# dashpay/agora-blsful

Measured on NVIDIA B200. Metric: verified sigs/sec, 1M-batch G2Impl, higher is better.
Workload: dtype u32 limbs (381-bit modular integers)

## Files before the change

### agora-blsful_b200/csrc/blsgpu.cu

```cuda
#include <cuda_runtime.h>
#include <nvtx3/nvToolsExt.h>
#include <sys/random.h>

#include <algorithm>
#include <atomic>
#include <functional>
#include <cstdio>
#include <cstdlib>
#include <cstring>
#include <memory>
#include <mutex>
#include <string>
#include <unordered_map>
#include <thread>
#include <vector>

#include "../../include/blsgpu.h"
#include "kernels.cuh"

using namespace bls;

namespace {

thread_local std::string g_create_error;
// ... 770 lines not shown
  return BLSGPU_OK;
}

template <class PkA, class SigA>
size_t pipeline_other_bytes(size_t n) {
  typedef typename PtInfo<SigA>::Jac SigJ;
  size_t total = levels_total(make_levels(std::max<size_t>(n, 1)));
  size_t gtotal = levels_total(make_levels((std::max<size_t>(n, 1) + M6_GROUP - 1) / M6_GROUP));
  return gtotal * (sizeof(Fp12) + sizeof(SigJ)) + n * (sizeof(SigJ) + sizeof(Fp12) + sizeof(SigJ)) + total * sizeof(Digest) +
         n * (16 + 4 * 32) + ((size_t)32 << 16) * (12 + 2 * sizeof(SigJ)) + (1 << 20) + (n + 64) * 8 + 16 * 256 + 4096 +
         probe_scratch_bytes<PkA, SigA>(probe_cap((n + M6_GROUP - 1) / M6_GROUP)) +
         (n >= MSM_MIN_ITEMS ? (n / 96 + 2) * 32 * sizeof(SigJ) + std::min<size_t>(n / 384 + 1, 592) * 128 * NODE_BUCKETS * sizeof(SigJ) + n * 5 + 8 * 256 : 0);
}
size_t m6_line_bytes(size_t n, size_t chunk) {
  return (n > chunk ? 2 : 1) * std::max<size_t>(std::min(std::max<size_t>(n, 1), chunk), 6 * PROBE_SMALL) * M6_ITEM_BYTES;
}
int ensure_miller_arena(blsgpu_ctx* ctx, size_t n, size_t other) {
  plan_m6_chunk(ctx, n, other);
  for (;;) {
    const int r = ensure_arena(ctx, other + m6_line_bytes(n, ctx->m6_chunk));
    if (r != BLSGPU_E_ALLOC || ctx->m6_chunk <= M6_CHUNK_MIN || n <= M6_CHUNK_MIN) return r;
    (void)cudaGetLastError();
    ctx->m6_chunk = std::max(M6_CHUNK_MIN, std::min(ctx->m6_chunk, n) / 2 / 120 * 120);
  }
}
template <class PkA, class SigA>
int ensure_pipeline_arena(blsgpu_ctx* ctx, size_t n, size_t head_bytes) {
  return ensure_miller_arena(ctx, n, head_bytes + pipeline_other_bytes<PkA, SigA>(n));
}

template <class A>
int decode_points(blsgpu_ctx* ctx, size_t n, const uint8_t* d_in, int format, A* d_out, uint8_t* d_st, int kid = -1) {
  LAUNCH_TIMED(kid, (k_decode<A>), blocks_for(n), TPB, n, d_in, format, d_out, d_st);
  LAUNCH_TIMED(kid < 0 ? -1 : kid + 1, (k_subgroup_check<A>), blocks_for(n), TPB, n, d_out, d_st);
  return BLSGPU_OK;
}

struct Keys {
  const uint8_t* bytes = nullptr;
  KeySet* set = nullptr;
  const uint32_t* idx = nullptr;
  Keys(const uint8_t* b = nullptr) : bytes(b) {}
  Keys(KeySet* s, const uint32_t* i) : set(s), idx(i) {}
};
template <class PkA>
int load_keys(blsgpu_ctx* ctx, size_t n, const Keys& d_keys, int format, PkA* d_pk, uint8_t* d_st) {
  if (!d_keys.set) return decode_points<PkA>(ctx, n, d_keys.bytes, format, d_pk, d_st, BLSGPU_KERNEL_DECODE_PK);
  LAUNCH((k_gather_keys<PkA>), blocks_for(n), TPB, n, d_keys.idx, (const PkA*)d_keys.set->pts, (const uint8_t*)d_keys.set->st, d_pk, d_st);
  return BLSGPU_OK;
}

template <class HA, class PkA>
int hash_points(blsgpu_ctx* ctx, size_t n, const uint8_t* d_msgs, const uint64_t* d_moff, int msg_mode, const PkA* d_pk,
                const uint8_t* d_pre, const DstParam& dst, HA* d_h) {
  typedef typename PtInfo<HA>::Jac HJ;
  size_t mark = ctx->arena.off;
  HJ* d_hj = ctx->arena.take<HJ>(n);
  if (ctx->arena.off > ctx->arena.cap) {
    ctx->err = "hash_points: arena too small";
    return BLSGPU_E_ALLOC;
  }
  LAUNCH_TIMED(BLSGPU_KERNEL_HASH_MAP, (k_hash<HA, PkA>), blocks_for(n), TPB, n, d_msgs, d_moff, msg_mode, d_pk, d_pre, dst, d_hj);
  LAUNCH_TIMED(BLSGPU_KERNEL_CLEAR_COFACTOR, (k_clear_cofactor<HA>), blocks_for(n), TPB, n, d_hj);
  LAUNCH_TIMED(BLSGPU_KERNEL_TO_AFFINE, (k_to_affine_batch<HA>), blocks_for((n + TO_AFFINE_BATCH - 1) / TO_AFFINE_BATCH), TPB, n,
               (const HJ*)d_hj, d_h);
  ctx->arena.off = mark;
  return BLSGPU_OK;
}

template <int IMPL>
int verify_points_partials(blsgpu_ctx* ctx, Pipe<typename ImplT<IMPL>::PkAff, typename ImplT<IMPL>::SigAff>& P, int msg_mode, const DstParam& dst,
                           size_t n, const typename ImplT<IMPL>::PkAff* d_pk, const typename ImplT<IMPL>::SigAff* d_sig, const uint8_t* d_stpk,
                           const uint8_t* d_stsig, const uint8_t* d_msgs, const uint64_t* d_moff, uint8_t* d_status_out) {
  typedef typename ImplT<IMPL>::PkAff PkA;
  typedef typename ImplT<IMPL>::SigAff SigA;
  SigA* d_h = ctx->arena.take<SigA>(n);
  LAUNCH((k_prestatus<PkA, SigA>), blocks_for(n), TPB, n, d_stpk, d_stsig, d_pk, d_sig, d_status_out);
  stage_mark(ctx, BLSGPU_STAGE_HASH);
  CKR((hash_points<SigA, PkA>(ctx, n, d_msgs, d_moff, msg_mode, d_pk, (const uint8_t*)d_status_out, dst, d_h)));
  return pipeline_partials<PkA, SigA>(ctx, P, n, d_pk, d_sig, d_h, d_status_out, true);
}
template <int IMPL>
int verify_points(blsgpu_ctx* ctx, int msg_mode, const DstParam& dst, size_t n, const typename ImplT<IMPL>::PkAff* d_pk,
                  const typename ImplT<IMPL>::SigAff* d_sig, const uint8_t* d_stpk, const uint8_t* d_stsig, const uint8_t* d_msgs,
                  const uint64_t* d_moff, uint8_t* d_status_out) {
  typedef typename ImplT<IMPL>::PkAff PkA;
  typedef typename ImplT<IMPL>::SigAff SigA;
  Pipe<PkA, SigA> P;
  CKR((verify_points_partials<IMPL>(ctx, P, msg_mode, dst, n, d_pk, d_sig, d_stpk, d_stsig, d_msgs, d_moff, d_status_out)));
  return check_and_bisect(ctx, P);
}

template <int IMPL>
int verify_dev_partials(blsgpu_ctx* ctx, Pipe<typename ImplT<IMPL>::PkAff, typename ImplT<IMPL>::SigAff>& P, int msg_mode, const DstParam& dst,
                        int format, size_t n, const Keys& d_keys, const uint8_t* d_sigs, const uint8_t* d_msgs, const uint64_t* d_moff,
                        uint8_t* d_status_out) {
// ... 2612 lines not shown
```

### agora-blsful_b200/csrc/kernels.cuh

```cuda
#pragma once
#include <cuda_runtime.h>

#include "h2c.cuh"
#include "pairing.cuh"
#include "miller6.cuh"
#include "finalexp6.cuh"
#include "fr.cuh"

namespace bls {

template <class A>
struct PtInfo;
template <>
struct PtInfo<G1Aff> {
  static const int LEN = 48;
  typedef G1Jac Jac;
  typedef Fp F;
};
template <>
struct PtInfo<G2Aff> {
  static const int LEN = 96;
  typedef G2Jac Jac;
  typedef Fp2 F;
};
__device__ __forceinline__ uint8_t pt_decompress(G1Aff& r, const uint8_t* b, bool chk) { return g1_decompress(r, b, chk); }
__device__ __forceinline__ uint8_t pt_decompress(G2Aff& r, const uint8_t* b, bool chk) { return g2_decompress(r, b, chk); }
__device__ __forceinline__ void pt_compress(uint8_t* o, const G1Aff& p) { g1_compress(o, p); }
__device__ __forceinline__ void pt_compress(uint8_t* o, const G2Aff& p) { g2_compress(o, p); }
__device__ __forceinline__ void pt_generator(G1Aff& g) {
  fp_set(g.x, K_G1X);
  fp_set(g.y, K_G1Y);
  g.inf = 0;
}
__device__ __forceinline__ void pt_generator(G2Aff& g) {
  fp2_set(g.x, K_G2X);
  fp2_set(g.y, K_G2Y);
  g.inf = 0;
}
template <class A>
__device__ __forceinline__ void pt_set_inf(A& p) {
  fzero(p.x);
  fzero(p.y);
  p.inf = 1;
}

template <int IMPL>
struct ImplT;
template <>
struct ImplT<2> {
  typedef G1Aff PkAff;
  typedef G2Aff SigAff;
  typedef G1Jac PkJac;
  typedef G2Jac SigJac;
};
template <>
struct ImplT<1> {
  typedef G2Aff PkAff;
  typedef G1Aff SigAff;
  typedef G2Jac PkJac;
  typedef G1Jac SigJac;
};
__device__ __forceinline__ void hash_to_group(G2Jac& r, const uint8_t* pre, uint32_t pl, const uint8_t* m, uint32_t ml,
                                              const uint8_t* dst, uint32_t dl) {
  hash_to_g2(r, pre, pl, m, ml, dst, dl);
}
__device__ __forceinline__ void hash_to_group(G1Jac& r, const uint8_t* pre, uint32_t pl, const uint8_t* m, uint32_t ml,
                                              const uint8_t* dst, uint32_t dl) {
  hash_to_g1(r, pre, pl, m, ml, dst, dl);
}

__device__ __forceinline__ void hash_map_to_curve(G2Jac& r, const uint8_t* pre, uint32_t pl, const uint8_t* m, uint32_t ml,
                                                  const uint8_t* dst, uint32_t dl) {
  hash_map_g2(r, pre, pl, m, ml, dst, dl);
}
__device__ __forceinline__ void hash_map_to_curve(G1Jac& r, const uint8_t* pre, uint32_t pl, const uint8_t* m, uint32_t ml,
                                                  const uint8_t* dst, uint32_t dl) {
  hash_map_g1(r, pre, pl, m, ml, dst, dl);
}
__device__ __forceinline__ void clear_cofactor(G2Jac& r, const G2Jac& q) { g2_clear_cofactor(r, q); }
__device__ __forceinline__ void clear_cofactor(G1Jac& r, const G1Jac& q) { g1_clear_cofactor(r, q); }

struct DstParam {
  uint8_t b[64];
  uint32_t len;
};
struct Digest {
  uint8_t b[32];
};

#define BLS_TID() ((size_t)blockIdx.x * blockDim.x + threadIdx.x)
#ifndef BLS_MIN_BLOCKS
#define BLS_MIN_BLOCKS 1
#endif

#if !defined(BLS_SPLIT_MIN_BLOCKS)
#define BLS_SPLIT_MIN_BLOCKS 4
#endif
#if !defined(BLS_HASH_MIN_BLOCKS)
#define BLS_HASH_MIN_BLOCKS 3
#endif
#if !defined(BLS_SPLIT2_MIN_BLOCKS)
#define BLS_SPLIT2_MIN_BLOCKS 4
#endif
template <class A>
struct SplitBlocks {
  static constexpr int value = sizeof(A) > 2 * sizeof(Fp) + 16 ? BLS_SPLIT2_MIN_BLOCKS : BLS_SPLIT_MIN_BLOCKS;
};
#if !defined(BLS_MSM_MIN_BLOCKS)
#define BLS_MSM_MIN_BLOCKS 4
#endif
template <class A>
__global__ void __launch_bounds__(128, BLS_MIN_BLOCKS) k_decode(size_t n, const uint8_t* __restrict__ in, int format, A* __restrict__ out,
                                                uint8_t* __restrict__ st) {
  constexpr int L = PtInfo<A>::LEN;
  __shared__ __align__(16) uint8_t stage[128 * L];
  const size_t first = (size_t)blockIdx.x * blockDim.x;
  const size_t cnt = first < n ? (n - first < blockDim.x ? n - first : blockDim.x) : 0;
  const uint8_t* src = in + first * L;
  if ((reinterpret_cast<uintptr_t>(src) & 15u) == 0) {
    const uint4* v = reinterpret_cast<const uint4*>(src);
    uint4* d = reinterpret_cast<uint4*>(stage);
    const size_t quads = cnt * L / 16, tail = cnt * L - quads * 16;
    for (size_t q = threadIdx.x; q < quads; q += blockDim.x) d[q] = v[q];
    if (threadIdx.x < tail) stage[quads * 16 + threadIdx.x] = src[quads * 16 + threadIdx.x];
  } else {
    for (size_t b = threadIdx.x; b < cnt * L; b += blockDim.x) stage[b] = src[b];
  }
  __syncthreads();
  size_t i = BLS_TID();
  if (i >= n) return;
  uint8_t b[L];
  const uint32_t* rec = reinterpret_cast<const uint32_t*>(stage + threadIdx.x * L);
#pragma unroll
  for (int k = 0; k < L / 4; k++) {
    uint32_t w = rec[k];
    b[4 * k] = (uint8_t)w;
    b[4 * k + 1] = (uint8_t)(w >> 8);
    b[4 * k + 2] = (uint8_t)(w >> 16);
    b[4 * k + 3] = (uint8_t)(w >> 24);
  }
  uint8_t s = header_to_modern(b[0], format);
  A p;
  if (s == ST_OK) s = pt_decompress(p, b, false);
  if (s != ST_OK) pt_set_inf(p);
  out[i] = p;
  st[i] = s;
}

__device__ __forceinline__ bool pt_in_subgroup(const G1Aff& p) { return g1_in_subgroup(p); }
__device__ __forceinline__ bool pt_in_subgroup(const G2Aff& p) { return g2_in_subgroup(p); }
template <class A>
__global__ void __launch_bounds__(128, SplitBlocks<A>::value) k_subgroup_check(size_t n, A* __restrict__ pts, uint8_t* __restrict__ st) {
  size_t i = BLS_TID();
  if (i >= n || st[i] != ST_OK) return;
  A p = pts[i];
  if (p.inf || pt_in_subgroup(p)) return;
  pt_set_inf(p);
  pts[i] = p;
  st[i] = ST_DESERIALIZE;
}

template <class A>
__global__ void __launch_bounds__(128, BLS_MIN_BLOCKS) k_gather_keys(size_t n, const uint32_t* __restrict__ key_idx, const A* __restrict__ set_pts,
                                                     const uint8_t* __restrict__ set_st, A* __restrict__ out, uint8_t* __restrict__ st) {
  size_t i = BLS_TID();
  if (i >= n) return;
  const uint32_t k = key_idx[i];
  out[i] = set_pts[k];
  st[i] = set_st[k];
}

template <class A>
__global__ void __launch_bounds__(128, BLS_MIN_BLOCKS) k_encode(size_t n, const A* __restrict__ in, int format, uint8_t* __restrict__ out) {
  size_t i = BLS_TID();
  if (i >= n) return;
  constexpr int L = PtInfo<A>::LEN;
  uint8_t b[L];
  A p = in[i];
  pt_compress(b, p);
  header_from_modern(b[0], format);
  for (int k = 0; k < L; k++) out[i * L + k] = b[k];
}

template <class A>
__global__ void __launch_bounds__(128, BLS_MIN_BLOCKS) k_to_affine(size_t n, const typename PtInfo<A>::Jac* __restrict__ in, A* __restrict__ out) {
  size_t i = BLS_TID();
  if (i >= n) return;
  typename PtInfo<A>::Jac p = in[i];
  A a;
  jac_to_aff(a, p);
  out[i] = a;
}

#define TO_AFFINE_BATCH 16
template <class A>
__global__ void __launch_bounds__(128) k_to_affine_batch(size_t n, const typename PtInfo<A>::Jac* __restrict__ in, A* __restrict__ out) {
  size_t base = BLS_TID() * TO_AFFINE_BATCH;
  if (base >= n) return;
  size_t left = n - base;
  jac_to_aff_batch<typename PtInfo<A>::F, TO_AFFINE_BATCH>(out + base, in + base, left < TO_AFFINE_BATCH ? (int)left : TO_AFFINE_BATCH);
}

template <class PkA, class SigA>
__global__ void k_prestatus(size_t n, const uint8_t* st_pk, const uint8_t* st_sig, const PkA* pk, const SigA* sig,
                            uint8_t* out) {
  size_t i = BLS_TID();
  if (i >= n) return;
  uint8_t s = st_pk[i];
  if (s == ST_OK) s = st_sig[i];
  if (s == ST_OK && sig[i].inf) s = ST_SIG_IDENTITY;
  if (s == ST_OK && pk[i].inf) s = ST_PK_IDENTITY;
  out[i] = s;
}

template <class HA, class PkA>
__global__ void __launch_bounds__(128, BLS_HASH_MIN_BLOCKS) k_hash(size_t n, const uint8_t* __restrict__ msgs, const uint64_t* __restrict__ msg_off,
                                              int msg_mode, const PkA* __restrict__ pk, const uint8_t* __restrict__ pre,
                                              DstParam dst, typename PtInfo<HA>::Jac* __restrict__ out) {
  size_t i = BLS_TID();
  if (i >= n) return;
  typename PtInfo<HA>::Jac hj;
  if (pre != nullptr && pre[i] != ST_OK) {
    jac_set_inf(hj);
    out[i] = hj;
    return;
  }
  uint8_t prefix[PtInfo<PkA>::LEN];
  uint32_t plen = 0;
  if (msg_mode != 0) {
    PkA p = pk[i];
    pt_compress(prefix, p);
    plen = PtInfo<PkA>::LEN;
  }
  const uint8_t* m = msgs;
  uint32_t mlen = 0;
  if (msg_mode != 2) {
    uint64_t o0 = msg_off[i], o1 = msg_off[i + 1];
    m = msgs + o0;
    mlen = (uint32_t)(o1 - o0);
  }
  hash_map_to_curve(hj, prefix, plen, m, mlen, dst.b, dst.len);
  out[i] = hj;
}

template <class HA>
__global__ void __launch_bounds__(128, SplitBlocks<HA>::value) k_clear_cofactor(size_t n, typename PtInfo<HA>::Jac* __restrict__ pts) {
  size_t i = BLS_TID();
  if (i >= n) return;
  typename PtInfo<HA>::Jac q = pts[i], r;
  if (jac_is_inf(q)) return;
  clear_cofactor(r, q);
  pts[i] = r;
}

template <class P>
__device__ __forceinline__ void digest_point(Sha256& s, const P& p) {
  sha256_update(s, reinterpret_cast<const uint8_t*>(&p.x), sizeof(p.x));
  sha256_update(s, reinterpret_cast<const uint8_t*>(&p.y), sizeof(p.y));
  const uint8_t f = p.inf ? 1 : 0;
  sha256_update(s, &f, 1);
}
template <class PkA, class SigA>
__global__ void __launch_bounds__(128, BLS_MIN_BLOCKS) k_leaf_digest(size_t n, const PkA* pk, const SigA* sig, const SigA* h, Digest* out) {
  size_t i = BLS_TID();
  if (i >= n) return;
  Sha256 s;
  sha256_init(s);
  digest_point(s, pk[i]);
  digest_point(s, sig[i]);
  digest_point(s, h[i]);
  Digest d;
  sha256_final(s, d.b);
  out[i] = d;
}
__global__ void __launch_bounds__(128, BLS_MIN_BLOCKS) k_digest_reduce(size_t n_in, const Digest* in, size_t n_out, Digest* out) {
  size_t j = BLS_TID();
  if (j >= n_out) return;
  Sha256 s;
  sha256_init(s);
  for (int m = 0; m < 16; m++) {
    size_t idx = j + (size_t)m * n_out;
    if (idx < n_in) sha256_update(s, in[idx].b, 32);
  }
  Digest d;
  sha256_final(s, d.b);
// ... 460 lines not shown
__global__ void __launch_bounds__(128, BLS_MIN_BLOCKS) k_reduce_jac_w(size_t n_in, const J* __restrict__ in, size_t n_out, J* __restrict__ out) {
  const size_t t = BLS_TID(), j = t >> 4;
  const int m = (int)(t & 15);
  const size_t idx = j + (size_t)m * n_out;
  J acc;
  if (j < n_out && idx < n_in) acc = in[idx]; else jac_set_inf(acc);
#pragma unroll 1
  for (int s = 1; s < 16; s <<= 1) {
    J other;
    words_shfl_xor(other, acc, s);
    if ((m & (2 * s - 1)) == 0) jac_add(acc, acc, other);
  }
  if (j < n_out && m == 0) out[j] = acc;
}
template <class A>
__global__ void __launch_bounds__(128, BLS_MIN_BLOCKS) k_reduce_aff(size_t n_in, const A* __restrict__ in, size_t n_out,
                                                    typename PtInfo<A>::Jac* __restrict__ out) {
  size_t j = BLS_TID();
  if (j >= n_out) return;
  typename PtInfo<A>::Jac acc;
  jac_set_inf(acc);
  for (int m = 0; m < 16; m++) {
    size_t idx = j + (size_t)m * n_out;
    if (idx < n_in) {
      A t = in[idx];
      jac_add_mixed(acc, acc, t);
    }
  }
  out[j] = acc;
}

constexpr uint8_t PROBE_SKIP = 0xfe;
template <class PkA, class SigA>
__global__ void __launch_bounds__(128, BLS_MIN_BLOCKS) k_probe_fill_nodes(size_t cnt, const uint32_t* __restrict__ idx,
                                                          const typename PtInfo<SigA>::Jac* __restrict__ S, PkA* __restrict__ xpk,
                                                          SigA* __restrict__ xh, uint8_t* __restrict__ xpre) {
  size_t c = BLS_TID();
  if (c >= cnt) return;
  const size_t j = idx ? idx[c] : c;
  typename PtInfo<SigA>::Jac s = S[j];
  SigA sa;
  jac_to_aff(sa, s);
  PkA ng;
  pt_generator(ng);
  aff_neg(ng, ng);
  xpk[6 * c] = ng;
  xh[6 * c] = sa;
  xpre[6 * c] = sa.inf ? PROBE_SKIP : ST_OK;
  for (int m = 1; m < 6; m++) xpre[6 * c + m] = PROBE_SKIP;
}
template <class PkA, class SigA>
__global__ void __launch_bounds__(128, BLS_MIN_BLOCKS) k_probe_fill_leaves(size_t cnt, const uint32_t* __restrict__ idx, const PkA* __restrict__ pk,
                                                           const SigA* __restrict__ h, const SigA* __restrict__ sig,
                                                           const uint8_t* __restrict__ status, PkA* __restrict__ xpk,
                                                           SigA* __restrict__ xh, uint8_t* __restrict__ xpre) {
  size_t c = BLS_TID();
  if (c >= cnt) return;
  const size_t i = idx[c];
  const bool on = status[i] == ST_OK;
  if (on) {
    PkA ng;
    pt_generator(ng);
    aff_neg(ng, ng);
    xpk[6 * c] = pk[i];
    xh[6 * c] = h[i];
    xpk[6 * c + 1] = ng;
    xh[6 * c + 1] = sig[i];
// ... 798 lines not shown
```

### agora-blsful_b200/csrc/fp.cuh

```cuda
#pragma once
#include <stdint.h>

#if defined(__CUDACC__)
#define BLS_HD __device__ __forceinline__
#define BLS_FN __device__ __noinline__
#define BLS_CONST __device__ __constant__ const
#else
#define BLS_HD static inline
#define BLS_FN static
#define BLS_CONST static const
#endif

#include "consts_gen.h"

#if defined(BLS_TRACK)
#include <cstdio>
#include <cstdlib>
#include <execinfo.h>
#define BLS_REQ(cond, what)                                                                  \
  do {                                                                                       \
    if (!(cond)) {                                                                           \
      fprintf(stderr, "BLS_TRACK bound violation: %s (%s:%d)\n", what, __FILE__, __LINE__);  \
      void* bt_[24];                                                                         \
      int n_ = backtrace(bt_, 24);                                                           \
// ... 357 lines not shown
#pragma unroll
  for (int i = 0; i < NL; i++) r.l[i] = c ? a.l[i] : b.l[i];
  r.l[NL] = r.l[NL + 1] = 0;
#if defined(BLS_TRACK)
  r.vb = a.vb > b.vb ? a.vb : b.vb;
  r.lb = a.lb > b.lb ? a.lb : b.lb;
#endif
}

BLS_HD void fp_to_mont(Fp& r, const Fp& raw) {
  Fp r2;
  fp_set(r2, K_R2);
  fp_mul(r, raw, r2);
}
BLS_HD void fp_from_mont(Fp& raw, const Fp& a) {
  Fp one, t;
  fp_zero(one);
  one.l[0] = 1;
  TRK(one, 1.0, 1);
  fp_mul(t, a, one);
  fp_canon(raw, t);
}

BLS_HD bool raw_gt_half(const Fp& raw) {
  int32_t br = 0;
#pragma unroll
  for (int i = 0; i < NL; i++) {
    int32_t t = (int32_t)K_HALF_P28[i] - (int32_t)raw.l[i] + br;
    br = t >> 31;
  }
  return br != 0;
}

BLS_FN void fp_pow_fixed(Fp& r, const Fp& a, const uint32_t* e) {
  Fp tbl[16];
  fp_one(tbl[0]);
  fp_norm(tbl[1], a);
  for (int i = 2; i < 16; i++) fp_mul(tbl[i], tbl[i - 1], tbl[1]);
  Fp acc;
  fp_one(acc);
  bool started = false;
  for (int limb = 11; limb >= 0; limb--) {
    uint32_t w = e[limb];
    for (int nib = 7; nib >= 0; nib--) {
      uint32_t d = (w >> (4 * nib)) & 15u;
      if (started) {
#pragma unroll 1
        for (int k = 0; k < 4; k++) fp_sqr_inl(acc, acc);
        if (d) fp_mul_inl(acc, acc, tbl[d]);
      } else if (d) {
        acc = tbl[d];
        started = true;
      }
    }
  }
  r = acc;
}

BLS_HD void fp_inv(Fp& r, const Fp& a) { fp_pow_fixed(r, a, K_EXP_PM2); }

BLS_HD void fp_isqrt_pow(Fp& t, const Fp& a) { fp_pow_fixed(t, a, K_EXP_PM3D4); }

BLS_HD bool fp_sqrt(Fp& r, const Fp& a) {
  Fp t, s, chk;
  fp_isqrt_pow(t, a);
  fp_mul(s, t, a);
  fp_sqr(chk, s);
  r = s;
  return fp_eq(chk, a);
}

BLS_HD bool fp_from_be48_raw(Fp& raw, const uint8_t* b) {
#pragma unroll
  for (int i = 0; i < NL; i++) {
    uint64_t v = 0;
#pragma unroll
    for (int k = 0; k < 5; k++) {
      int byte_index = (28 * i) / 8 + k;
      if (byte_index < 48) v |= (uint64_t)b[47 - byte_index] << (8 * k);
    }
    raw.l[i] = (uint32_t)(v >> ((28 * i) % 8)) & M28;
  }
  raw.l[NL] = raw.l[NL + 1] = 0;
  TRK(raw, 1.0, M28);
  int32_t br = 0;
#pragma unroll
  for (int i = 0; i < NL; i++) {
    int32_t t = (int32_t)raw.l[i] - (int32_t)p28(i) + br;
    br = t >> 31;
  }
  return br != 0;
}
BLS_HD void fp_to_be48_raw(uint8_t* b, const Fp& raw) {
#pragma unroll
  for (int byte_index = 0; byte_index < 48; byte_index++) {
    int bit = 8 * byte_index;
    int i = bit / 28, sh = bit % 28;
    uint32_t v = raw.l[i] >> sh;
    if (sh > 20 && i + 1 < NL) v |= raw.l[i + 1] << (28 - sh);
    b[47 - byte_index] = (uint8_t)v;
  }
}
BLS_HD void fp_raw_from_words(Fp& raw, const uint32_t* w, int n) {
#pragma unroll
// ... 14 lines not shown
```

### agora-blsful_b200/csrc/fp2.cuh

```cuda
#pragma once
#include "fp.cuh"

namespace bls {

struct Fp2 {
  Fp c0, c1;
};

BLS_HD void fadd(Fp& r, const Fp& a, const Fp& b) { fp_add(r, a, b); }
template <int K>
BLS_HD void fsub_k(Fp& r, const Fp& a, const Fp& b) { fp_sub_k<K>(r, a, b); }
template <int K>
BLS_HD void fneg_k(Fp& r, const Fp& a) { fp_neg_k<K>(r, a); }
BLS_HD void fsub(Fp& r, const Fp& a, const Fp& b) {
  fp_sub_k<16>(r, a, b);
  fp_norm(r, r);
}
BLS_HD void fneg(Fp& r, const Fp& a) {
  fp_neg_k<16>(r, a);
  fp_norm(r, r);
}
BLS_HD void fdbl(Fp& r, const Fp& a) { fp_add(r, a, a); }
BLS_HD void fnorm(Fp& r, const Fp& a) { fp_norm(r, a); }
BLS_HD void fred(Fp& r, const Fp& a) { fp_red(r, a); }
BLS_HD void fmul(Fp& r, const Fp& a, const Fp& b) { fp_mul(r, a, b); }
BLS_HD void fsqr(Fp& r, const Fp& a) { fp_sqr(r, a); }
BLS_HD bool fis_zero(const Fp& a) { return fp_is_zero(a); }
BLS_HD bool feq(const Fp& a, const Fp& b) { return fp_eq(a, b); }
BLS_HD void fzero(Fp& r) { fp_zero(r); }
BLS_HD void fone(Fp& r) { fp_one(r); }
BLS_HD void fselect(Fp& r, bool c, const Fp& a, const Fp& b) { fp_select(r, c, a, b); }
BLS_HD void finv(Fp& r, const Fp& a) { fp_inv(r, a); }

BLS_HD void fp2_set(Fp2& r, const uint32_t (*c)[NL]) {
// ... 377 lines not shown
```

Measured before the change: 1.308 million.

## Split G2 subgroup check and cofactor clearing across two lanes per point

```diff
diff --git a/agora-blsful_b200/csrc/blsgpu.cu b/agora-blsful_b200/csrc/blsgpu.cu
--- a/agora-blsful_b200/csrc/blsgpu.cu
+++ b/agora-blsful_b200/csrc/blsgpu.cu
@@ -826,7 +826,7 @@
 template <class A>
 int decode_points(blsgpu_ctx* ctx, size_t n, const uint8_t* d_in, int format, A* d_out, uint8_t* d_st, int kid = -1) {
   LAUNCH_TIMED(kid, (k_decode<A>), blocks_for(n), TPB, n, d_in, format, d_out, d_st);
-  LAUNCH_TIMED(kid < 0 ? -1 : kid + 1, (k_subgroup_check<A>), blocks_for(n), TPB, n, d_out, d_st);
+  LAUNCH_TIMED(kid < 0 ? -1 : kid + 1, (k_subgroup_check<A>), blocks_for(n * PtInfo<A>::LANES), TPB, n, d_out, d_st);
   return BLSGPU_OK;
 }
 
@@ -855,7 +855,7 @@
     return BLSGPU_E_ALLOC;
   }
   LAUNCH_TIMED(BLSGPU_KERNEL_HASH_MAP, (k_hash<HA, PkA>), blocks_for(n), TPB, n, d_msgs, d_moff, msg_mode, d_pk, d_pre, dst, d_hj);
-  LAUNCH_TIMED(BLSGPU_KERNEL_CLEAR_COFACTOR, (k_clear_cofactor<HA>), blocks_for(n), TPB, n, d_hj);
+  LAUNCH_TIMED(BLSGPU_KERNEL_CLEAR_COFACTOR, (k_clear_cofactor<HA>), blocks_for(n * PtInfo<HA>::LANES), TPB, n, d_hj);
   LAUNCH_TIMED(BLSGPU_KERNEL_TO_AFFINE, (k_to_affine_batch<HA>), blocks_for((n + TO_AFFINE_BATCH - 1) / TO_AFFINE_BATCH), TPB, n,
                (const HJ*)d_hj, d_h);
   ctx->arena.off = mark;
diff --git a/agora-blsful_b200/csrc/g2lane.cuh b/agora-blsful_b200/csrc/g2lane.cuh
--- /dev/null
+++ b/agora-blsful_b200/csrc/g2lane.cuh
@@ -0,0 +1,462 @@
+#pragma once
+#include "sfp.cuh"
+
+namespace bls {
+
+struct alignas(16) LFp {
+  int32_t w[NL];
+#if defined(BLS_TRACK)
+  double vb, lb;
+#endif
+};
+struct L2Jac {
+  LFp X, Y, Z;
+};
+struct L2Aff {
+  LFp x, y;
+};
+
+#if !defined(__CUDA_ARCH__)
+int l2_host_lane();
+void l2_host_xchg(void* partner, const void* mine, unsigned bytes);
+#endif
+
+BLS_HD int l2_lane() {
+#if defined(__CUDA_ARCH__)
+  return (int)(threadIdx.x & 1u);
+#else
+  return l2_host_lane();
+#endif
+}
+BLS_HD void l2_xchg(LFp& p, const LFp& a) {
+#if defined(__CUDA_ARCH__)
+  const unsigned m = 3u << (threadIdx.x & 30u);
+#pragma unroll
+  for (int i = 0; i < NL; i++) p.w[i] = __shfl_xor_sync(m, a.w[i], 1);
+#else
+  l2_host_xchg(&p, &a, sizeof(LFp));
+#endif
+}
+BLS_HD bool l2_both(bool b) {
+#if defined(__CUDA_ARCH__)
+  const unsigned m = 3u << (threadIdx.x & 30u);
+  return b && __shfl_xor_sync(m, (int)b, 1) != 0;
+#else
+  int mine = b ? 1 : 0, other = 0;
+  l2_host_xchg(&other, &mine, sizeof(int));
+  return b && other != 0;
+#endif
+}
+
+#if defined(BLS_TRACK)
+#define LTRK(r, v, l) \
+  do {                \
+    (r).vb = (v);     \
+    (r).lb = (l);     \
+  } while (0)
+#else
+#define LTRK(r, v, l) \
+  do {                \
+  } while (0)
+#endif
+
+BLS_HD void l2_add(LFp& r, const LFp& a, const LFp& b) {
+#if defined(BLS_TRACK)
+  BLS_REQ(a.lb + b.lb < 2147483648.0 - 134217728.0, "l2_add limb overflow");
+  const double v_ = a.vb + b.vb, l_ = a.lb + b.lb;
+#endif
+#pragma unroll
+  for (int i = 0; i < NL; i++) r.w[i] = a.w[i] + b.w[i];
+  LTRK(r, v_, l_);
+}
+BLS_HD void l2_sub(LFp& r, const LFp& a, const LFp& b) {
+#if defined(BLS_TRACK)
+  BLS_REQ(a.lb + b.lb < 2147483648.0 - 134217728.0, "l2_sub limb overflow");
+  const double v_ = a.vb + b.vb, l_ = a.lb + b.lb;
+#endif
+#pragma unroll
+  for (int i = 0; i < NL; i++) r.w[i] = a.w[i] - b.w[i];
+  LTRK(r, v_, l_);
+}
+template <int K>
+BLS_HD void l2_smul(LFp& r, const LFp& a) {
+#if defined(BLS_TRACK)
+  BLS_REQ(K * a.lb < 2147483648.0 - 134217728.0, "l2_smul limb overflow");
+  const double v_ = K * a.vb, l_ = K * a.lb;
+#endif
+#pragma unroll
+  for (int i = 0; i < NL; i++) r.w[i] = K * a.w[i];
+  LTRK(r, v_, l_);
+}
+BLS_HD void l2_neg(LFp& r, const LFp& a) {
+#pragma unroll
+  for (int i = 0; i < NL; i++) r.w[i] = -a.w[i];
+  LTRK(r, a.vb, a.lb);
+}
+BLS_HD void l2_conj(LFp& r, const LFp& a) {
+  const int32_t s = l2_lane() ? -1 : 1;
+#pragma unroll
+  for (int i = 0; i < NL; i++) r.w[i] = s * a.w[i];
+  LTRK(r, a.vb, a.lb);
+}
+BLS_HD void l2_norm(LFp& r, const LFp& a) {
+  int32_t c[NL - 1];
+#pragma unroll
+  for (int i = 0; i < NL - 1; i++) c[i] = (a.w[i] + (1 << 27)) >> 28;
+  r.w[0] = a.w[0] - c[0] * (1 << 28);
+#pragma unroll
+  for (int i = 1; i < NL - 1; i++) r.w[i] = a.w[i] - c[i] * (1 << 28) + c[i - 1];
+  r.w[NL - 1] = a.w[NL - 1] + c[NL - 2];
+#if defined(BLS_TRACK)
+  BLS_REQ(a.lb < 2147483648.0 - 134217728.0 && a.vb < 1000.0, "l2_norm input");
+  LTRK(r, a.vb, 134217728.0 + (double)((uint64_t)a.lb >> 28) + 1.0);
+#endif
+}
+BLS_HD void l2_const(LFp& r, const uint32_t (*c)[NL]) {
+  const int h = l2_lane();
+#pragma unroll
+  for (int i = 0; i < NL; i++) r.w[i] = (int32_t)c[h][i];
+  LTRK(r, 1.0, 268435455.0);
+}
+BLS_HD void l2_one(LFp& r) {
+  const int h = l2_lane();
+#pragma unroll
+  for (int i = 0; i < NL; i++) r.w[i] = h ? 0 : (int32_t)K_ONE[i];
+  LTRK(r, 1.0, 268435455.0);
+}
+BLS_HD void l2_zero(LFp& r) {
+#pragma unroll
+  for (int i = 0; i < NL; i++) r.w[i] = 0;
+  LTRK(r, 0.0, 0.0);
+}
+
+BLS_HD void l2_from_fp(LFp& r, const Fp& a) {
+#pragma unroll
+  for (int i = 0; i < NL; i++) r.w[i] = (int32_t)a.l[i];
+#if defined(BLS_TRACK)
+  BLS_REQ(a.lb < (1u << 30), "l2_from_fp: limbs too large");
+  LTRK(r, a.vb, (double)a.lb);
+#endif
+  l2_norm(r, r);
+}
+BLS_HD void l2_to_fp(Fp& r, const LFp& a) {
+#if defined(BLS_TRACK)
+  BLS_REQ(a.vb < 250.0 && a.lb <= 1073741820.0, "l2_to_fp input");
+#endif
+#pragma unroll
+  for (int i = 0; i < NL; i++) r.l[i] = kps<256>(i) + (uint32_t)a.w[i];
+  r.l[NL] = r.l[NL + 1] = 0;
+  TRK(r, 256.0 + a.vb, (1ull << 30) + (1ull << 28) + (uint64_t)a.lb);
+}
+BLS_HD void l2_store(Fp& r, const LFp& a) {
+  Fp t;
+  l2_to_fp(t, a);
+  fp_red(r, t);
+}
+BLS_HD bool l2_is_zero(const LFp& a) {
+  Fp t;
+  l2_to_fp(t, a);
+  return l2_both(fp_is_zero(t));
+}
+
+#if defined(BLS_TRACK)
+BLS_HD void l2_req_prod(double la, double lb, int terms) {
+  const double lim = 9223372036854775808.0 - 15.0 * 72057594037927936.0;
+  BLS_REQ(la < 1073741824.0 && lb < 1073741824.0, "l2 product operand limbs");
+  BLS_REQ(14.0 * terms * la * lb < lim, "l2 product column overflow");
+}
+#endif
+BLS_HD void l2_redc_store(LFp& r, uint64_t* T) {
+  int32_t o[NL];
+  T[2 * NL - 1] = 0;
+  sop_redc(o, T);
+#pragma unroll
+  for (int i = 0; i < NL; i++) r.w[i] = o[i];
+}
+BLS_FN void l2_mul(LFp& r, const LFp& a, const LFp& b) {
+  LFp ap, bp;
+  l2_xchg(ap, a);
+  l2_xchg(bp, b);
+  const int h = l2_lane();
+#if defined(BLS_TRACK)
+  const double la = a.lb > ap.lb ? a.lb : ap.lb, lbb = b.lb > bp.lb ? b.lb : bp.lb;
+  const double va = a.vb > ap.vb ? a.vb : ap.vb, vbb = b.vb > bp.vb ? b.vb : bp.vb;
+  l2_req_prod(la, lbb, 2);
+  BLS_REQ(2.0 * va * vbb / 2500.0 + 1.0 < 4.0, "l2_mul result value bound");
+#endif
+  uint64_t T[2 * NL];
+  int32_t x[NL], y[NL];
+#pragma unroll
+  for (int i = 0; i < 2 * NL; i++) T[i] = 0;
+#pragma unroll
+  for (int i = 0; i < NL; i++) {
+    x[i] = a.w[i];
+    y[i] = h ? bp.w[i] : b.w[i];
+  }
+  sop_acc(T, x, y);
+#pragma unroll
+  for (int i = 0; i < NL; i++) {
+    x[i] = h ? ap.w[i] : -ap.w[i];
+    y[i] = h ? b.w[i] : bp.w[i];
+  }
+  sop_acc(T, x, y);
+  l2_redc_store(r, T);
+  LTRK(r, 2.0 * va * vbb / 2500.0 + 1.0, 134217728.0);
+}
+BLS_FN void l2_sqr(LFp& r, const LFp& a) {
+  LFp ap;
+  l2_xchg(ap, a);
+  const int h = l2_lane();
+#if defined(BLS_TRACK)
+  const double la = a.lb > ap.lb ? a.lb : ap.lb, va = a.vb > ap.vb ? a.vb : ap.vb;
+  l2_req_prod(2.0 * la, 2.0 * la, 1);
+  BLS_REQ(2.0 * va * va / 2500.0 + 1.0 < 4.0, "l2_sqr result value bound");
+#endif
+  uint64_t T[2 * NL];
+  int32_t x[NL], y[NL];
+#pragma unroll
+  for (int i = 0; i < 2 * NL; i++) T[i] = 0;
+#pragma unroll
+  for (int i = 0; i < NL; i++) {
+    x[i] = h ? 2 * ap.w[i] : a.w[i] + ap.w[i];
+    y[i] = h ? a.w[i] : a.w[i] - ap.w[i];
+  }
+  sop_acc(T, x, y);
+  l2_redc_store(r, T);
+  LTRK(r, 2.0 * va * va / 2500.0 + 1.0, 134217728.0);
+}
+BLS_HD void l2_mul_fpc(LFp& r, const LFp& a, const uint32_t* k) {
+#if defined(BLS_TRACK)
+  l2_req_prod(a.lb, 268435455.0, 1);
+#endif
+  uint64_t T[2 * NL];
+  int32_t x[NL], y[NL];
+#pragma unroll
+  for (int i = 0; i < 2 * NL; i++) T[i] = 0;
+#pragma unroll
+  for (int i = 0; i < NL; i++) {
+    x[i] = a.w[i];
+    y[i] = (int32_t)k[i];
+  }
+  sop_acc(T, x, y);
+  l2_redc_store(r, T);
+  LTRK(r, a.vb / 2500.0 + 1.0, 134217728.0);
+}
+
+BLS_HD void l2_set_inf(L2Jac& r) {
+  l2_one(r.X);
+  l2_one(r.Y);
+  l2_zero(r.Z);
+}
+BLS_HD void l2_from_aff(L2Jac& r, const L2Aff& p) {
+  r.X = p.x;
+  r.Y = p.y;
+  l2_one(r.Z);
+}
+
+BLS_FN void l2_dbl(L2Jac& r, const L2Jac& p) {
+  LFp t0, t1, t2, t3;
+  l2_mul(t0, p.Y, p.Z);
+  l2_sqr(t1, p.Y);
+  l2_add(t2, p.X, t1);
+  l2_sqr(t2, t2);
+  l2_sqr(t3, p.X);
+  l2_sqr(t1, t1);
+  l2_sub(t2, t2, t3);
+  l2_sub(t2, t2, t1);
+  l2_norm(t2, t2);
+  l2_add(t0, t0, t0);
+  l2_norm(r.Z, t0);
+  l2_add(t0, t3, t3);
+  l2_add(t0, t0, t3);
+  l2_norm(t0, t0);
+  l2_sqr(t3, t0);
+  l2_smul<4>(r.X, t2);
+  l2_sub(r.X, t3, r.X);
+  l2_norm(r.X, r.X);
+  l2_add(t2, t2, t2);
+  l2_sub(t2, t2, r.X);
+  l2_mul(t3, t0, t2);
+  l2_smul<8>(t1, t1);
+  l2_sub(t3, t3, t1);
+  l2_norm(r.Y, t3);
+}
+
+BLS_FN void l2_add_mixed(L2Jac& r, const L2Jac& p, const L2Aff& q) {
+  if (l2_is_zero(p.Z)) {
+    l2_from_aff(r, q);
+    return;
+  }
+  LFp a, b, c, d, e, f, g, h;
+  l2_sqr(a, p.Z);
+  l2_mul(b, q.x, a);
+  l2_mul(c, q.y, p.Z);
+  l2_mul(c, c, a);
+  l2_sub(b, b, p.X);
+  l2_norm(b, b);
+  l2_sub(c, c, p.Y);
+  l2_norm(c, c);
+  if (l2_is_zero(b)) {
+    if (l2_is_zero(c)) {
+      l2_dbl(r, p);
+    } else {
+      l2_set_inf(r);
+    }
+    return;
+  }
+  l2_add(c, c, c);
+  l2_sqr(d, b);
+  l2_smul<4>(e, d);
+  l2_mul(f, b, e);
+  l2_mul(e, p.X, e);
+  l2_sqr(g, c);
+  l2_add(h, e, e);
+  l2_add(h, h, f);
+  l2_sub(g, g, h);
+  l2_norm(g, g);
+  l2_sub(e, e, g);
+  l2_mul(e, c, e);
+  l2_mul(f, p.Y, f);
+  l2_add(f, f, f);
+  l2_sub(e, e, f);
+  l2_add(h, p.Z, b);
+  l2_sqr(h, h);
+  l2_add(a, a, d);
+  l2_sub(h, h, a);
+  l2_norm(r.Y, e);
+  r.X = g;
+  l2_norm(r.Z, h);
+}
+
+BLS_FN void l2_add_jac(L2Jac& r, const L2Jac& p, const L2Jac& q) {
+  if (l2_is_zero(q.Z)) {
+    r = p;
+    return;
+  }
+  if (l2_is_zero(p.Z)) {
+    r = q;
+    return;
+  }
+  LFp a, b, c, d, e, f, g, h, i;
+  l2_sqr(a, p.Z);
+  l2_sqr(b, q.Z);
+  l2_mul(c, p.X, b);
+  l2_mul(d, q.X, a);
+  l2_mul(e, p.Y, q.Z);
+  l2_mul(e, e, b);
+  l2_mul(f, q.Y, p.Z);
+  l2_mul(f, f, a);
+  l2_sub(d, d, c);
+  l2_norm(d, d);
+  l2_sub(f, f, e);
+  l2_norm(f, f);
+  if (l2_is_zero(d)) {
+    if (l2_is_zero(f)) {
+      l2_dbl(r, p);
+    } else {
+      l2_set_inf(r);
+    }
+    return;
+  }
+  l2_add(f, f, f);
+  l2_add(g, d, d);
+  l2_sqr(g, g);
+  l2_mul(h, d, g);
+  l2_mul(c, c, g);
+  l2_sqr(g, f);
+  l2_add(i, c, c);
+  l2_add(i, i, h);
+  l2_sub(g, g, i);
+  l2_norm(g, g);
+  l2_sub(c, c, g);
+  l2_mul(c, f, c);
+  l2_mul(e, e, h);
+  l2_add(e, e, e);
+  l2_sub(c, c, e);
+  l2_add(i, p.Z, q.Z);
+  l2_sqr(i, i);
+  l2_add(a, a, b);
+  l2_sub(i, i, a);
+  l2_norm(i, i);
+  l2_mul(i, i, d);
+  l2_norm(r.Y, c);
+  r.X = g;
+  r.Z = i;
+}
+
+BLS_HD void l2_mul_xabs(L2Jac& r, const L2Jac& p) {
+  r = p;
+  const uint64_t e = K_X_ABS;
+  for (int i = 62; i >= 0; i--) {
+    l2_dbl(r, r);
+    if ((e >> i) & 1) l2_add_jac(r, r, p);
+  }
+}
+BLS_HD void l2_mul_xabs_aff(L2Jac& r, const L2Aff& p) {
+  l2_from_aff(r, p);
+  const uint64_t e = K_X_ABS;
+  for (int i = 62; i >= 0; i--) {
+    l2_dbl(r, r);
+    if ((e >> i) & 1) l2_add_mixed(r, r, p);
+  }
+}
+
+BLS_FN void l2_psi(L2Jac& r, const L2Jac& p) {
+  LFp c, t;
+  l2_const(c, K_PSI_CX);
+  l2_conj(t, p.X);
+  l2_mul(r.X, t, c);
+  l2_const(c, K_PSI_CY);
+  l2_conj(t, p.Y);
+  l2_mul(r.Y, t, c);
+  l2_conj(r.Z, p.Z);
+}
+BLS_HD void l2_psi2(L2Jac& r, const L2Jac& p) {
+  l2_mul_fpc(r.X, p.X, K_PSI2_CX);
+  l2_neg(r.Y, p.Y);
+  r.Z = p.Z;
+}
+
+BLS_FN bool l2_in_subgroup(const L2Aff& p) {
+  L2Jac t;
+  l2_mul_xabs_aff(t, p);
+  if (l2_is_zero(t.Z)) return false;
+  LFp c, u, z2;
+  l2_const(c, K_PSI_CX);
+  l2_conj(u, p.x);
+  l2_mul(u, u, c);
+  l2_sqr(z2, t.Z);
+  l2_mul(u, u, z2);
+  l2_sub(u, u, t.X);
+  if (!l2_is_zero(u)) return false;
+  l2_const(c, K_PSI_CY);
+  l2_conj(u, p.y);
+  l2_mul(u, u, c);
+  l2_mul(z2, z2, t.Z);
+  l2_mul(u, u, z2);
+  l2_add(u, u, t.Y);
+  return l2_is_zero(u);
+}
+
+template <class Load>
+BLS_HD void l2_clear_cofactor(L2Jac& r, const Load& load) {
+  L2Jac u;
+  load(u);
+  l2_mul_xabs(r, u);
+  load(u);
+  l2_psi(u, u);
+  l2_neg(r.Y, r.Y);
+  l2_add_jac(u, u, r);
+  l2_mul_xabs(r, u);
+  l2_add_jac(r, r, u);
+  load(u);
+  L2Jac t;
+  l2_dbl(t, u);
+  l2_psi2(t, t);
+  l2_neg(u.Y, u.Y);
+  l2_add_jac(t, t, u);
+  l2_neg(r.Y, r.Y);
+  l2_add_jac(r, t, r);
+}
+
+}
diff --git a/agora-blsful_b200/csrc/kernels.cuh b/agora-blsful_b200/csrc/kernels.cuh
--- a/agora-blsful_b200/csrc/kernels.cuh
+++ b/agora-blsful_b200/csrc/kernels.cuh
@@ -6,6 +6,7 @@
 #include "miller6.cuh"
 #include "finalexp6.cuh"
 #include "fr.cuh"
+#include "g2lane.cuh"
 
 namespace bls {
 
@@ -14,12 +15,14 @@
 template <>
 struct PtInfo<G1Aff> {
   static const int LEN = 48;
+  static const int LANES = 1;
   typedef G1Jac Jac;
   typedef Fp F;
 };
 template <>
 struct PtInfo<G2Aff> {
   static const int LEN = 96;
+  static const int LANES = 2;
   typedef G2Jac Jac;
   typedef Fp2 F;
 };
@@ -77,8 +80,6 @@
                                                   const uint8_t* dst, uint32_t dl) {
   hash_map_g1(r, pre, pl, m, ml, dst, dl);
 }
-__device__ __forceinline__ void clear_cofactor(G2Jac& r, const G2Jac& q) { g2_clear_cofactor(r, q); }
-__device__ __forceinline__ void clear_cofactor(G1Jac& r, const G1Jac& q) { g1_clear_cofactor(r, q); }
 
 struct DstParam {
   uint8_t b[64];
@@ -147,17 +148,29 @@
   st[i] = s;
 }
 
-__device__ __forceinline__ bool pt_in_subgroup(const G1Aff& p) { return g1_in_subgroup(p); }
-__device__ __forceinline__ bool pt_in_subgroup(const G2Aff& p) { return g2_in_subgroup(p); }
 template <class A>
 __global__ void __launch_bounds__(128, SplitBlocks<A>::value) k_subgroup_check(size_t n, A* __restrict__ pts, uint8_t* __restrict__ st) {
-  size_t i = BLS_TID();
-  if (i >= n || st[i] != ST_OK) return;
-  A p = pts[i];
-  if (p.inf || pt_in_subgroup(p)) return;
-  pt_set_inf(p);
-  pts[i] = p;
-  st[i] = ST_DESERIALIZE;
+  if constexpr (PtInfo<A>::LANES == 1) {
+    size_t i = BLS_TID();
+    if (i >= n || st[i] != ST_OK) return;
+    A p = pts[i];
+    if (p.inf || g1_in_subgroup(p)) return;
+    pt_set_inf(p);
+    pts[i] = p;
+    st[i] = ST_DESERIALIZE;
+  } else {
+    const size_t i = BLS_TID() >> 1;
+    if (i >= n || st[i] != ST_OK || pts[i].inf) return;
+    const int h = l2_lane();
+    L2Aff p;
+    l2_from_fp(p.x, h ? pts[i].x.c1 : pts[i].x.c0);
+    l2_from_fp(p.y, h ? pts[i].y.c1 : pts[i].y.c0);
+    if (l2_in_subgroup(p) || h) return;
+    A q;
+    pt_set_inf(q);
+    pts[i] = q;
+    st[i] = ST_DESERIALIZE;
+  }
 }
 
 template <class A>
@@ -245,12 +258,34 @@
 
 template <class HA>
 __global__ void __launch_bounds__(128, SplitBlocks<HA>::value) k_clear_cofactor(size_t n, typename PtInfo<HA>::Jac* __restrict__ pts) {
-  size_t i = BLS_TID();
-  if (i >= n) return;
-  typename PtInfo<HA>::Jac q = pts[i], r;
-  if (jac_is_inf(q)) return;
-  clear_cofactor(r, q);
-  pts[i] = r;
+  if constexpr (PtInfo<HA>::LANES == 1) {
+    size_t i = BLS_TID();
+    if (i >= n) return;
+    typename PtInfo<HA>::Jac q = pts[i], r;
+    if (jac_is_inf(q)) return;
+    g1_clear_cofactor(r, q);
+    pts[i] = r;
+  } else {
+    const size_t i = BLS_TID() >> 1;
+    if (i >= n) return;
+    const int h = l2_lane();
+    G2Jac* q = pts + i;
+    const auto load = [q, h](L2Jac& p) {
+      l2_from_fp(p.X, h ? q->X.c1 : q->X.c0);
+      l2_from_fp(p.Y, h ? q->Y.c1 : q->Y.c0);
+      l2_from_fp(p.Z, h ? q->Z.c1 : q->Z.c0);
+    };
+    {
+      L2Jac p;
+      load(p);
+      if (l2_is_zero(p.Z)) return;
+    }
+    L2Jac r;
+    l2_clear_cofactor(r, load);
+    l2_store(h ? q->X.c1 : q->X.c0, r.X);
+    l2_store(h ? q->Y.c1 : q->Y.c0, r.Y);
+    l2_store(h ? q->Z.c1 : q->Z.c0, r.Z);
+  }
 }
 
 template <class P>
```

Measured after the change: 1.340 million, median of 6. 2.4% higher.

## Run fixed-exponent Fp powering in FP64-FMA 50-bit limb Montgomery arithmetic

Applied to the files above, without the earlier changes.

```diff
diff --git a/agora-blsful_b200/csrc/fp.cuh b/agora-blsful_b200/csrc/fp.cuh
--- a/agora-blsful_b200/csrc/fp.cuh
+++ b/agora-blsful_b200/csrc/fp.cuh
@@ -413,44 +413,6 @@
   return br != 0;
 }
 
-BLS_FN void fp_pow_fixed(Fp& r, const Fp& a, const uint32_t* e) {
-  Fp tbl[16];
-  fp_one(tbl[0]);
-  fp_norm(tbl[1], a);
-  for (int i = 2; i < 16; i++) fp_mul(tbl[i], tbl[i - 1], tbl[1]);
-  Fp acc;
-  fp_one(acc);
-  bool started = false;
-  for (int limb = 11; limb >= 0; limb--) {
-    uint32_t w = e[limb];
-    for (int nib = 7; nib >= 0; nib--) {
-      uint32_t d = (w >> (4 * nib)) & 15u;
-      if (started) {
-#pragma unroll 1
-        for (int k = 0; k < 4; k++) fp_sqr_inl(acc, acc);
-        if (d) fp_mul_inl(acc, acc, tbl[d]);
-      } else if (d) {
-        acc = tbl[d];
-        started = true;
-      }
-    }
-  }
-  r = acc;
-}
-
-BLS_HD void fp_inv(Fp& r, const Fp& a) { fp_pow_fixed(r, a, K_EXP_PM2); }
-
-BLS_HD void fp_isqrt_pow(Fp& t, const Fp& a) { fp_pow_fixed(t, a, K_EXP_PM3D4); }
-
-BLS_HD bool fp_sqrt(Fp& r, const Fp& a) {
-  Fp t, s, chk;
-  fp_isqrt_pow(t, a);
-  fp_mul(s, t, a);
-  fp_sqr(chk, s);
-  r = s;
-  return fp_eq(chk, a);
-}
-
 BLS_HD bool fp_from_be48_raw(Fp& raw, const uint8_t* b) {
 #pragma unroll
   for (int i = 0; i < NL; i++) {
diff --git a/agora-blsful_b200/csrc/fp2.cuh b/agora-blsful_b200/csrc/fp2.cuh
--- a/agora-blsful_b200/csrc/fp2.cuh
+++ b/agora-blsful_b200/csrc/fp2.cuh
@@ -1,5 +1,5 @@
 #pragma once
-#include "fp.cuh"
+#include "fpd.cuh"
 
 namespace bls {
 
diff --git a/agora-blsful_b200/csrc/fpd.cuh b/agora-blsful_b200/csrc/fpd.cuh
--- /dev/null
+++ b/agora-blsful_b200/csrc/fpd.cuh
@@ -0,0 +1,330 @@
+#pragma once
+#include "fp.cuh"
+
+#if !defined(__CUDACC__)
+#include <cmath>
+#include <cstring>
+#endif
+
+namespace bls {
+
+constexpr int ND = 8;
+constexpr uint64_t M50 = (1ull << 50) - 1;
+
+struct alignas(16) Fpd {
+  double l[ND];
+#if defined(BLS_TRACK)
+  double vb;
+  double lb;
+#endif
+};
+
+BLS_HD constexpr uint64_t pd50(int i) {
+  constexpr uint64_t t[ND] = {0x2ffffffffaaabull, 0x3ac54ffffee7full, 0x30f6241eabfffull, 0x2fd9cc34a83daull,
+                              0x0774b84f38512ull, 0x1ed90d2eb35d9ull, 0x397fe69a4b1baull, 0x00000680447a8ull};
+  return t[i];
+}
+constexpr uint64_t K_PINV50 = 0x3fffcfffcfffdull;
+BLS_HD constexpr uint64_t k2e408(int i) {
+  constexpr uint64_t t[ND] = {0x203480ea898baull, 0x309f24a23e874ull, 0x12aee547c6b37ull, 0x01b776e1bb031ull,
+                              0x2c4609523d536ull, 0x3e82e37aa4cdfull, 0x1b838ba6bf713ull, 0x00000630f33bdull};
+  return t[i];
+}
+BLS_HD constexpr uint64_t k2e392(int i) {
+  constexpr uint64_t t[ND] = {0x000000347fcb8ull, 0x39b4800ac4676ull, 0x090c7212e00cdull, 0x380dd9a7e0e88ull,
+                              0x1b09b42da0f73ull, 0x17663c4a5eec2ull, 0x3cfa012ca7c51ull, 0x0000015de9967ull};
+  return t[i];
+}
+
+constexpr double D2E50 = 0x1p50;
+constexpr double D2E52 = 0x1p52;
+constexpr double D2E102 = 0x1p102;
+constexpr double D2E102P52 = 0x1p102 + 0x1p52;
+constexpr uint64_t B2E52 = 0x4330000000000000ull;
+constexpr uint64_t B2E102 = 0x4650000000000000ull;
+
+BLS_HD uint64_t dbits(double x) {
+#if defined(__CUDA_ARCH__)
+  return (uint64_t)__double_as_longlong(x);
+#else
+  uint64_t v;
+  memcpy(&v, &x, 8);
+  return v;
+#endif
+}
+BLS_HD double bitsd(uint64_t v) {
+#if defined(__CUDA_ARCH__)
+  return __longlong_as_double((long long)v);
+#else
+  double x;
+  memcpy(&x, &v, 8);
+  return x;
+#endif
+}
+BLS_HD double u52_to_d(uint64_t v) {
+#if defined(__CUDA_ARCH__)
+  return __dsub_rn(bitsd(B2E52 | v), D2E52);
+#else
+  return bitsd(B2E52 | v) - D2E52;
+#endif
+}
+BLS_HD uint64_t d_to_u52(double x) {
+#if defined(__CUDA_ARCH__)
+  return dbits(__dadd_rn(x, D2E52)) - B2E52;
+#else
+  return dbits(x + D2E52) - B2E52;
+#endif
+}
+BLS_HD double d_twice(double x) {
+#if defined(__CUDA_ARCH__)
+  return __dadd_rn(x, x);
+#else
+  return x + x;
+#endif
+}
+
+BLS_HD void fpd_split(uint64_t& hi, uint64_t& lo, double a, double b) {
+#if defined(__CUDA_ARCH__)
+  const double t = __fma_rz(a, b, D2E102);
+  const double l = __fma_rn(a, b, __dsub_rn(D2E102P52, t));
+#else
+  double t = std::fma(a, b, D2E102);
+  if (std::fma(a, b, D2E102 - t) < 0) t = std::nextafter(t, 0.0);
+  const double l = std::fma(a, b, D2E102P52 - t);
+#endif
+  hi = dbits(t) - B2E102;
+  lo = dbits(l) - B2E52;
+#if defined(BLS_TRACK)
+  BLS_REQ(t >= D2E102 && t < 2.0 * D2E102, "fpd_split: high half left its binade");
+  BLS_REQ(l >= D2E52 && l < D2E52 + D2E50, "fpd_split: low half out of range");
+  const unsigned __int128 x = (unsigned __int128)(uint64_t)a * (uint64_t)b;
+  BLS_REQ(hi == (uint64_t)(x >> 50) && lo == ((uint64_t)x & M50), "fpd_split: halves differ from the integer product");
+#endif
+}
+
+#if defined(BLS_TRACK)
+#define FPD_COLS_REQ(cb)                                                                          \
+  do {                                                                                               \
+    for (int k_ = 0; k_ < 2 * ND; k_++) BLS_REQ((cb)[k_] < 9.2e18, "fpd column sum overflow");        \
+  } while (0)
+#endif
+
+BLS_HD void fpd_redc(Fpd& r, uint64_t* c
+#if defined(BLS_TRACK)
+                     , double* cb, double vprod
+#endif
+) {
+#pragma unroll
+  for (int i = 0; i < ND; i++) {
+    const uint64_t m = (c[i] * K_PINV50) & M50;
+    const double md = u52_to_d(m);
+#pragma unroll
+    for (int j = 0; j < ND; j++) {
+      uint64_t hi, lo;
+      fpd_split(hi, lo, md, (double)pd50(j));
+      c[i + j] += lo;
+      c[i + j + 1] += hi;
+#if defined(BLS_TRACK)
+      cb[i + j] += D2E50;
+      cb[i + j + 1] += D2E50;
+#endif
+    }
+#if defined(BLS_TRACK)
+    BLS_REQ((c[i] & M50) == 0, "fpd_redc: row not divisible by 2^50");
+    cb[i + 1] += cb[i] / D2E50;
+#endif
+    c[i + 1] += c[i] >> 50;
+  }
+#if defined(BLS_TRACK)
+  FPD_COLS_REQ(cb);
+  double cmax = 0;
+  for (int k = ND; k < 2 * ND - 1; k++) cmax = cb[k] > cmax ? cb[k] : cmax;
+  r.lb = D2E50 + cmax / D2E50;
+  r.vb = 1.0 + vprod * 4.0e114 / 2.58e120;
+  BLS_REQ(r.vb < 2.0, "fpd_redc: value >= 2p, limb 7 could exceed 2^33");
+#endif
+#pragma unroll
+  for (int k = 0; k < ND; k++) {
+    uint64_t v = k == ND - 1 ? c[ND + k] : (c[ND + k] & M50);
+    if (k > 0) v += c[ND + k - 1] >> 50;
+    r.l[k] = u52_to_d(v);
+  }
+}
+
+BLS_HD void fpd_mul_inl(Fpd& r, const Fpd& a, const Fpd& b) {
+#if defined(BLS_TRACK)
+  BLS_REQ(a.lb * b.lb < D2E102, "fpd_mul: limb product >= 2^102");
+  BLS_REQ(a.vb * b.vb < 16.0, "fpd_mul: value bound");
+  double cb[2 * ND];
+  for (int k = 0; k < 2 * ND; k++) cb[k] = 0;
+  for (int i = 0; i < ND; i++)
+    for (int j = 0; j < ND; j++) {
+      cb[i + j] += D2E50;
+      cb[i + j + 1] += a.lb * b.lb / D2E50;
+    }
+  FPD_COLS_REQ(cb);
+#endif
+  uint64_t c[2 * ND];
+#pragma unroll
+  for (int k = 0; k < 2 * ND; k++) c[k] = 0;
+#pragma unroll
+  for (int i = 0; i < ND; i++) {
+#pragma unroll
+    for (int j = 0; j < ND; j++) {
+      uint64_t hi, lo;
+      fpd_split(hi, lo, a.l[i], b.l[j]);
+      c[i + j] += lo;
+      c[i + j + 1] += hi;
+    }
+  }
+#if defined(BLS_TRACK)
+  fpd_redc(r, c, cb, a.vb * b.vb);
+#else
+  fpd_redc(r, c);
+#endif
+}
+
+BLS_HD void fpd_sqr_inl(Fpd& r, const Fpd& a) {
+#if defined(BLS_TRACK)
+  BLS_REQ(2.0 * a.lb * a.lb < D2E102, "fpd_sqr: doubled limb product >= 2^102");
+  BLS_REQ(a.vb * a.vb < 16.0, "fpd_sqr: value bound");
+  double cb[2 * ND];
+  for (int k = 0; k < 2 * ND; k++) cb[k] = 0;
+  for (int i = 0; i < ND; i++)
+    for (int j = i; j < ND; j++) {
+      cb[i + j] += D2E50;
+      cb[i + j + 1] += (i == j ? 1.0 : 2.0) * a.lb * a.lb / D2E50;
+    }
+  FPD_COLS_REQ(cb);
+#endif
+  double a2[ND];
+#pragma unroll
+  for (int j = 1; j < ND; j++) a2[j] = d_twice(a.l[j]);
+  uint64_t c[2 * ND];
+#pragma unroll
+  for (int k = 0; k < 2 * ND; k++) c[k] = 0;
+#pragma unroll
+  for (int i = 0; i < ND; i++) {
+    uint64_t hi, lo;
+    fpd_split(hi, lo, a.l[i], a.l[i]);
+    c[2 * i] += lo;
+    c[2 * i + 1] += hi;
+#pragma unroll
+    for (int j = i + 1; j < ND; j++) {
+      fpd_split(hi, lo, a.l[i], a2[j]);
+      c[i + j] += lo;
+      c[i + j + 1] += hi;
+    }
+  }
+#if defined(BLS_TRACK)
+  fpd_redc(r, c, cb, a.vb * a.vb);
+#else
+  fpd_redc(r, c);
+#endif
+}
+
+BLS_FN void fpd_mul(Fpd& r, const Fpd& a, const Fpd& b) { fpd_mul_inl(r, a, b); }
+
+BLS_HD void fpd_set_u50(Fpd& r, const uint64_t* v) {
+#pragma unroll
+  for (int k = 0; k < ND; k++) r.l[k] = u52_to_d(v[k]);
+#if defined(BLS_TRACK)
+  r.vb = 1.0;
+  r.lb = D2E50;
+#endif
+}
+
+BLS_HD void fpd_from_fp(Fpd& r, const Fp& a) {
+#if defined(BLS_TRACK)
+  BLS_REQ(a.lb < (1ull << 32) && a.vb < 2000.0, "fpd_from_fp: input outside the lazy bounds");
+#endif
+  uint32_t x[NL];
+  fp_red_inl(x, a);
+  uint64_t v[ND], k[ND];
+#pragma unroll
+  for (int j = 0; j < ND; j++) {
+    uint64_t w = 0;
+#pragma unroll
+    for (int i = 0; i < NL; i++) {
+      const int sh = 28 * i - 50 * j;
+      if (sh >= 0 && sh < 50) w |= (uint64_t)x[i] << sh;
+      else if (sh < 0 && sh > -28) w |= (uint64_t)x[i] >> -sh;
+    }
+    v[j] = w & M50;
+    k[j] = k2e408(j);
+  }
+  Fpd raw, kk;
+  fpd_set_u50(raw, v);
+#if defined(BLS_TRACK)
+  raw.vb = 3.0;
+#endif
+  fpd_set_u50(kk, k);
+  fpd_mul(r, raw, kk);
+}
+
+BLS_HD void fp_from_fpd(Fp& r, const Fpd& a) {
+  uint64_t k[ND];
+#pragma unroll
+  for (int j = 0; j < ND; j++) k[j] = k2e392(j);
+  Fpd kk, t;
+  fpd_set_u50(kk, k);
+  fpd_mul(t, a, kk);
+  uint64_t y[ND], c = 0;
+#pragma unroll
+  for (int j = 0; j < ND; j++) {
+    c += d_to_u52(t.l[j]);
+    y[j] = j == ND - 1 ? c : (c & M50);
+    c >>= 50;
+  }
+  Fp x;
+#pragma unroll
+  for (int i = 0; i < NL; i++) {
+    const int bit = 28 * i, j = bit / 50, sh = bit % 50;
+    uint64_t w = y[j] >> sh;
+    if (sh > 22 && j + 1 < ND) w |= y[j + 1] << (50 - sh);
+    x.l[i] = i == NL - 1 ? (uint32_t)w : (uint32_t)w & M28;
+  }
+  x.l[NL] = x.l[NL + 1] = 0;
+  TRK(x, 2.0, M28);
+  fp_canon(r, x);
+}
+
+BLS_FN void fp_pow_fixed(Fp& r, const Fp& a, const uint32_t* e) {
+  Fpd tbl[16];
+  fpd_from_fp(tbl[1], a);
+#pragma unroll 1
+  for (int i = 2; i < 16; i++) fpd_mul(tbl[i], tbl[i - 1], tbl[1]);
+  Fpd acc = tbl[1];
+  bool started = false;
+  for (int limb = 11; limb >= 0; limb--) {
+    uint32_t w = e[limb];
+    for (int nib = 7; nib >= 0; nib--) {
+      uint32_t d = (w >> (4 * nib)) & 15u;
+      if (started) {
+#pragma unroll 1
+        for (int k = 0; k < 4; k++) fpd_sqr_inl(acc, acc);
+        if (d) fpd_mul_inl(acc, acc, tbl[d]);
+      } else if (d) {
+        acc = tbl[d];
+        started = true;
+      }
+    }
+  }
+  if (started) fp_from_fpd(r, acc);
+  else fp_one(r);
+}
+
+BLS_HD void fp_inv(Fp& r, const Fp& a) { fp_pow_fixed(r, a, K_EXP_PM2); }
+
+BLS_HD void fp_isqrt_pow(Fp& t, const Fp& a) { fp_pow_fixed(t, a, K_EXP_PM3D4); }
+
+BLS_HD bool fp_sqrt(Fp& r, const Fp& a) {
+  Fp t, s, chk;
+  fp_isqrt_pow(t, a);
+  fp_mul(s, t, a);
+  fp_sqr(chk, s);
+  r = s;
+  return fp_eq(chk, a);
+}
+
+}
diff --git a/agora-blsful_b200/csrc/kernels.cuh b/agora-blsful_b200/csrc/kernels.cuh
--- a/agora-blsful_b200/csrc/kernels.cuh
+++ b/agora-blsful_b200/csrc/kernels.cuh
@@ -99,6 +99,12 @@
 #if !defined(BLS_HASH_MIN_BLOCKS)
 #define BLS_HASH_MIN_BLOCKS 3
 #endif
+#if !defined(BLS_CHAIN_MIN_BLOCKS)
+#define BLS_CHAIN_MIN_BLOCKS 3
+#endif
+#if !defined(BLS_CHAIN4_MIN_BLOCKS)
+#define BLS_CHAIN4_MIN_BLOCKS 4
+#endif
 #if !defined(BLS_SPLIT2_MIN_BLOCKS)
 #define BLS_SPLIT2_MIN_BLOCKS 4
 #endif
@@ -110,7 +116,7 @@
 #define BLS_MSM_MIN_BLOCKS 4
 #endif
 template <class A>
-__global__ void __launch_bounds__(128, BLS_MIN_BLOCKS) k_decode(size_t n, const uint8_t* __restrict__ in, int format, A* __restrict__ out,
+__global__ void __launch_bounds__(128, BLS_CHAIN_MIN_BLOCKS) k_decode(size_t n, const uint8_t* __restrict__ in, int format, A* __restrict__ out,
                                                 uint8_t* __restrict__ st) {
   constexpr int L = PtInfo<A>::LEN;
   __shared__ __align__(16) uint8_t stage[128 * L];
@@ -183,7 +189,7 @@
 }
 
 template <class A>
-__global__ void __launch_bounds__(128, BLS_MIN_BLOCKS) k_to_affine(size_t n, const typename PtInfo<A>::Jac* __restrict__ in, A* __restrict__ out) {
+__global__ void __launch_bounds__(128, BLS_CHAIN4_MIN_BLOCKS) k_to_affine(size_t n, const typename PtInfo<A>::Jac* __restrict__ in, A* __restrict__ out) {
   size_t i = BLS_TID();
   if (i >= n) return;
   typename PtInfo<A>::Jac p = in[i];
@@ -777,7 +783,7 @@
 
 constexpr uint8_t PROBE_SKIP = 0xfe;
 template <class PkA, class SigA>
-__global__ void __launch_bounds__(128, BLS_MIN_BLOCKS) k_probe_fill_nodes(size_t cnt, const uint32_t* __restrict__ idx,
+__global__ void __launch_bounds__(128, BLS_CHAIN4_MIN_BLOCKS) k_probe_fill_nodes(size_t cnt, const uint32_t* __restrict__ idx,
                                                           const typename PtInfo<SigA>::Jac* __restrict__ S, PkA* __restrict__ xpk,
                                                           SigA* __restrict__ xh, uint8_t* __restrict__ xpre) {
   size_t c = BLS_TID();
```

Result: faster. 1.310 million before, 1.323 million after (median of 6 runs) (+1.0%).
